# crowsonkb/k-diffusion

Hardware: NVIDIA H100
Metric: images/sec (256x256, Heun 50-step) (higher is better)
Workload: dtype bf16

## Files before the change

__graft_entry__.py:

```python
import os
import subprocess
import sys
from pathlib import Path

ROOT = Path(__file__).resolve().parent
PKG = ROOT / "k-diffusion_b200"
for p in (str(ROOT), str(PKG)):
    if p not in sys.path:
        sys.path.insert(0, p)


def build():
    env = dict(os.environ)
    env["PATH"] = os.path.join(env.get("CUDA_HOME", "/usr/local/cuda"), "bin") + os.pathsep + env.get("PATH", "")
    subprocess.run(["make", "-C", str(PKG / "csrc"), "-j8"], check=True, env=env)
    import k_diffusion
    from k_diffusion import _native
    lib = _native.lib()
    assert lib.kdb_abi_version() == _native.ABI_VERSION
    print(f"built {_native.LIB_PATH} (ABI {_native.ABI_VERSION}, {len(_native.SIGNATURES)} symbols bound)")


def smoke():
    import json
# ... 4 lines not shown
    from oracle import kdiff_oracle as O
    from oracle.fixtures import assert_close, synth_sd

    assert torch.cuda.is_available(), "smoke() needs a GPU"
    meta = json.loads((ROOT / "tests/golden/cfg1_mnist_shapes.json").read_text())
    cfg = K.config.load_config(meta["config"])
    sd = synth_sd(meta["shapes"], 1)
    inner = K.config.make_model(cfg)
    inner.load_state_dict(sd)
    inner = inner.to("cuda:0").eval().set_precision("fp32")
    model = K.config.make_denoiser_wrapper(cfg)(inner)
    g = torch.Generator().manual_seed(0)
    x = torch.randn(2, 1, 28, 28, generator=g) * 80
    cc = torch.tensor([3, 10])
    sigmas = K.sampling.get_sigmas_karras(3, 1e-2, 80)
    want = O.sample_heun(O.make_denoiser(sd, cfg["model"]), x, sigmas, dict(class_cond=cc))
    n0 = K.sampling.total_kernel_launches()
    got = K.sampling.sample_heun(model, x.cuda(), sigmas.cuda(), extra_args=dict(class_cond=cc.cuda()), disable=True)
    torch.cuda.synchronize()
    assert_close(got, want, what="smoke: sample_heun vs oracle")
    inner.set_precision("bf16")
    b = model(x.cuda(), torch.tensor([1.0, 5.0], device="cuda"), class_cond=cc.cuda())
    assert torch.isfinite(b).all()
    meta = json.loads((ROOT / "tests/golden/sw64_shapes.json").read_text())
    budget = json.loads((ROOT / "tests/golden/bf16_budget.json").read_text())["sw64_heun6"]["rel_l2"]
    cfg2 = K.config.load_config(meta["config"])
    sd2 = synth_sd(meta["shapes"], 1)
    inner2 = K.config.make_model(cfg2)
    inner2.load_state_dict(sd2)
    model2 = K.config.make_denoiser_wrapper(cfg2)(inner2.to("cuda:0").eval().set_precision("bf16"))
    g = torch.Generator().manual_seed(124)
# ... 15 lines not shown
```

k-diffusion_b200/csrc/tc_common.cuh:

```cuda
#pragma once
#include <cuda.h>

#include "common.cuh"
#include "pipe_state.cuh"

namespace kdb {
namespace tc {

__device__ __forceinline__ uint32_t smem_u32(const void* p) { return (uint32_t)__cvta_generic_to_shared(p); }

__device__ __forceinline__ void pdl_wait() { asm volatile("griddepcontrol.wait;" ::: "memory"); }

__device__ __forceinline__ uint8_t* smem_1k() {
  extern __shared__ uint8_t smem_raw[];
  return reinterpret_cast<uint8_t*>((reinterpret_cast<uintptr_t>(smem_raw) + 1023) & ~(uintptr_t)1023);
}
__device__ __forceinline__ int tiles_owned(int tiles) {
  return (int)blockIdx.x < tiles ? (tiles - 1 - (int)blockIdx.x) / (int)gridDim.x + 1 : 0;
}

__device__ __forceinline__ void mbar_init(uint64_t* bar, uint32_t count) {
  asm volatile("mbarrier.init.shared::cta.b64 [%0], %1;" ::"r"(smem_u32(bar)), "r"(count));
}
__device__ __forceinline__ void fence_barrier_init() { asm volatile("fence.mbarrier_init.release.cluster;" ::: "memory"); }
// ... 43 lines not shown
                   smem_u32(smem_dst)),
               "l"(reinterpret_cast<uint64_t>(map)), "r"(smem_u32(bar)), "r"(c0), "r"(c1), "r"(c2)
               : "memory");
}
__device__ __forceinline__ void tma_load_4d(void* smem_dst, const CUtensorMap* map, uint64_t* bar, int c0, int c1, int c2, int c3) {
  asm volatile("cp.async.bulk.tensor.4d.shared::cluster.global.mbarrier::complete_tx::bytes [%0], [%1, {%3, %4, %5, %6}], [%2];" ::"r"(
                   smem_u32(smem_dst)),
               "l"(reinterpret_cast<uint64_t>(map)), "r"(smem_u32(bar)), "r"(c0), "r"(c1), "r"(c2), "r"(c3)
               : "memory");
}

__device__ __forceinline__ void tma_load_5d(void* smem_dst, const CUtensorMap* map, uint64_t* bar, int c0, int c1, int c2, int c3, int c4) {
  asm volatile("cp.async.bulk.tensor.5d.shared::cluster.global.mbarrier::complete_tx::bytes [%0], [%1, {%3, %4, %5, %6, %7}], [%2];" ::"r"(
                   smem_u32(smem_dst)),
               "l"(reinterpret_cast<uint64_t>(map)), "r"(smem_u32(bar)), "r"(c0), "r"(c1), "r"(c2), "r"(c3), "r"(c4)
               : "memory");
}
__device__ __forceinline__ void tma_store_4d(const CUtensorMap* map, const void* smem_src, int c0, int c1, int c2, int c3) {
  asm volatile("cp.async.bulk.tensor.4d.global.shared::cta.bulk_group [%0, {%2, %3, %4, %5}], [%1];" ::"l"(reinterpret_cast<uint64_t>(map)),
               "r"(smem_u32(smem_src)), "r"(c0), "r"(c1), "r"(c2), "r"(c3)
               : "memory");
}
__device__ __forceinline__ void tma_store_3d(const CUtensorMap* map, const void* smem_src, int c0, int c1, int c2) {
  asm volatile("cp.async.bulk.tensor.3d.global.shared::cta.bulk_group [%0, {%2, %3, %4}], [%1];" ::"l"(reinterpret_cast<uint64_t>(map)),
               "r"(smem_u32(smem_src)), "r"(c0), "r"(c1), "r"(c2)
               : "memory");
}
__device__ __forceinline__ void tma_store_2d(const CUtensorMap* map, const void* smem_src, int c0, int c1) {
  asm volatile("cp.async.bulk.tensor.2d.global.shared::cta.bulk_group [%0, {%2, %3}], [%1];" ::"l"(reinterpret_cast<uint64_t>(map)),
               "r"(smem_u32(smem_src)), "r"(c0), "r"(c1)
// ... 160 lines not shown
      "{\n\t.reg .pred p;\n\t"
      "elect.sync _|p, 0xffffffff;\n\t"
      "selp.u32 %0, 1, 0, p;\n\t}"
      : "=r"(pred));
  return pred != 0;
}

__device__ __forceinline__ uint32_t pack_bf16x2(float lo, float hi) {
  __nv_bfloat162 t = __floats2bfloat162_rn(lo, hi);
  return *reinterpret_cast<uint32_t*>(&t);
}
__device__ __forceinline__ void unpack_bf16x2(uint32_t v, float& lo, float& hi) {
  __nv_bfloat162 t = *reinterpret_cast<__nv_bfloat162*>(&v);
  lo = __low2float(t);
  hi = __high2float(t);
}

__device__ __forceinline__ void window_coords(int win, int h, int w, int& b, int& wi, int& wj) {
  const int nww = w >> 3, per_img = (h >> 3) * nww;
  b = win / per_img;
  const int rem = win - b * per_img;
  wi = rem / nww;
  wj = rem - wi * nww;
}
__device__ __forceinline__ void quad_origin(int wi, int wj, int q, int h, int w, int shift, int& r, int& c) {
  r = (wi * 8 + (q >> 1) * 4 - shift + h) % h;
  c = (wj * 8 + (q & 1) * 4 - shift + w) % w;
}
__device__ __forceinline__ bool seam_ok(int qq, int kq, bool seam_r, bool seam_c) {
  return (!seam_r || ((kq >> 1) == (qq >> 1))) && (!seam_c || ((kq & 1) == (qq & 1)));
// ... 129 lines not shown
```

k-diffusion_b200/csrc/tc_ffn_fused.cuh:

```cuda
#pragma once

constexpr int FF_C = 128;
constexpr int FF_CH = 64;
constexpr int FF_XBUF = 2, FF_WU = 3, FF_WD = 3;
constexpr int FF_X_BYTES = 2 * A_STAGE_BYTES;
constexpr int FF_WU_BYTES = 2 * A_STAGE_BYTES;
constexpr int FF_WD_BYTES = A_STAGE_BYTES;
constexpr int FF_THREADS = 256 + 128;

struct FfnBars {
  tc::TmaRing<FF_XBUF> x;
  tc::TmaRing<FF_WU> wu;
  tc::TmaRing<FF_WD> wd;
};
constexpr size_t FF_SMEM = (size_t)FF_XBUF * FF_X_BYTES + (size_t)FF_WU * FF_WU_BYTES + (size_t)FF_WD * FF_WD_BYTES + sizeof(FfnBars) + 1024;

struct FfnParams {
  const float* ss_in;
  float* ss_out;
  int64_t M;
  int nc;
};

__global__ void __launch_bounds__(FF_THREADS, 1) ffn_fused_kernel(const __grid_constant__ CUtensorMap tmx, const __grid_constant__ CUtensorMap tmwu,
// ... 64 lines not shown
    const uint32_t xa = tc::smem_u32(sX + (size_t)xs.slot * FF_X_BYTES) + (uint32_t)wg * 8192u;
#pragma unroll
    for (int j = 0; j < 64; ++j) acc2[j] = 0.f;
    for (int c = 0; c <= nc; ++c) {
      if (c > 0) {
        tc::wg_wait<0>();
        tc::wg_fence_acc(acc1);
        tc::wg_fence_acc(acc2);
        tc::wg_fence_acc(hreg);
        if (lane == 0) bars->wu.release(us);
        us.advance();
        if (c > 1) {
          if (lane == 0) bars->wd.release(ds);
          ds.advance();
        }
#pragma unroll
        for (int q = 0; q < 8; ++q) {
          const tc::f32x2 v0 = tc::mul2(tc::pk2(acc1[8 * q], acc1[8 * q + 1]), h0), v1 = tc::mul2(tc::pk2(acc1[8 * q + 2], acc1[8 * q + 3]), h1);
          const tc::f32x2 q0 = tc::mul2(tc::pk2(acc1[8 * q + 4], acc1[8 * q + 5]), g0), q1 = tc::mul2(tc::pk2(acc1[8 * q + 6], acc1[8 * q + 7]), g1);
          float o0, o1, o2, o3;
          tc::upk2(tc::geglu2(v0, q0), o0, o1);
          tc::upk2(tc::geglu2(v1, q1), o2, o3);
          hreg[(q >> 1) * 4 + (q & 1) * 2 + 0] = tc::pack_bf16x2(o0, o1);
          hreg[(q >> 1) * 4 + (q & 1) * 2 + 1] = tc::pack_bf16x2(o2, o3);
        }
      }
#pragma unroll
      for (int j = 0; j < 64; ++j) acc1[j] = 0.f;
      tc::wg_fence_acc(acc1);
      if (wg == 1) tc::named_barrier_sync(tc::BAR_TURN + 1, 256);
      else if (!first_block) tc::named_barrier_sync(tc::BAR_TURN, 256);
      first_block = false;
      if (c > 0) {
        bars->wd.wait(ds);
        const uint64_t bd = tc::smem_desc_k_sw128(wd_base + ds.slot * (uint32_t)FF_WD_BYTES);
        tc::wg_fence_acc(acc2);
        tc::wg_fence_acc(hreg);
        tc::wg_fence();
#pragma unroll
        for (int kk = 0; kk < 4; ++kk) {
// ... 61 lines not shown
```

k-diffusion_b200/csrc/tc_kernels.cu:

```cuda
#include "tc_common.cuh"
#include "tc_kernels.cuh"

namespace kdb {

typedef CUresult (*EncodeTiledFn)(CUtensorMap*, CUtensorMapDataType, cuuint32_t, void*, const cuuint64_t*, const cuuint64_t*,
                                  const cuuint32_t*, const cuuint32_t*, CUtensorMapInterleave, CUtensorMapSwizzle,
                                  CUtensorMapL2promotion, CUtensorMapFloatOOBfill);

static EncodeTiledFn encode_fn() {
  static EncodeTiledFn fn = [] {
    void* p = nullptr;
    cudaDriverEntryPointQueryResult q;
    if (cudaGetDriverEntryPoint("cuTensorMapEncodeTiled", &p, cudaEnableDefault, &q) != cudaSuccess) p = nullptr;
    return reinterpret_cast<EncodeTiledFn>(p);
  }();
  return fn;
}

int make_tmap_bf16(CUtensorMap* out, const void* base, int rank, const uint64_t* dims, const uint64_t* strides_bytes, const uint32_t* box) {
  EncodeTiledFn fn = encode_fn();
  KDB_REQUIRE(fn != nullptr, KDB_ERR_UNSUPPORTED, "cuTensorMapEncodeTiled not available from this driver");
  cuuint64_t gd[5];
  cuuint64_t gs[5];
  cuuint32_t bx[5], es[5];
// ... 20 lines not shown

bool pdl_enabled() {
  static const bool enabled = [] {
    const char* e = getenv("KDB200_NO_PDL");
    return !(e != nullptr && e[0] == '1');
  }();
  return enabled;
}

namespace {

constexpr int BM = 128, BK = 64;
constexpr int A_STAGE_BYTES = BM * BK * 2;
constexpr int SUB_TILE_BYTES = BM * 128;
constexpr int GEMM_THREADS = 384;
constexpr int GEMM_RING_BYTES = 96 * 1024;

struct GemmArgs : GemmEpi {
  bf16* out;
  int64_t M;
  int N, K;
  int box_w, box_h;
  int th, tw;
};

__device__ __forceinline__ float bf16_round(float v) { return __bfloat162float(__float2bfloat16_rn(v)); }

int tmap_2d(CUtensorMap* t, const void* base, uint64_t inner, uint64_t outer, uint32_t box_inner, uint32_t box_outer) {
  const uint64_t dims[2] = {inner, outer};
  const uint64_t strides[1] = {inner * 2};
  const uint32_t box[2] = {box_inner, box_outer};
// ... 8 lines not shown
}

bool quad_box(int wc, int* box_w, int* box_h) {
  if (wc >= BM) {
    if (wc % BM != 0) return false;
    *box_w = BM;
    *box_h = 1;
    return true;
  }
  if (BM % wc != 0) return false;
  *box_w = wc;
  *box_h = BM / wc;
  return true;
}

template <int BN, int EPI> constexpr int out_bytes() {
  return EPI == EPI_GEGLU ? SUB_TILE_BYTES : (EPI == EPI_SPLIT_LERP || EPI == EPI_PATCH_OUT) ? 0 : (BN / 64) * SUB_TILE_BYTES;
}
template <int BN, int EPI> constexpr size_t gemm_smem() { return 1024 + GEMM_RING_BYTES + BM * BN * 4 + 2 * out_bytes<BN, EPI>() + 128; }

template <int BN> __device__ __forceinline__ int stage_off(int row, int chunk) { return row * BN + ((chunk ^ (row & 7)) << 2); }
template <int BN>
__device__ __forceinline__ void stage_store(float* s, int row0, const float (&d)[BN / 2]) {
  const int t = threadIdx.x & 127;
  const int r = row0 + 16 * (t >> 5) + ((t & 31) >> 2), c = 2 * (t & 3);
#pragma unroll
  for (int j = 0; j < BN / 8; ++j) {
    *reinterpret_cast<float2*>(s + stage_off<BN>(r, 2 * j + (c >> 2)) + (c & 3)) = make_float2(d[4 * j], d[4 * j + 1]);
    *reinterpret_cast<float2*>(s + stage_off<BN>(r + 8, 2 * j + (c >> 2)) + (c & 3)) = make_float2(d[4 * j + 2], d[4 * j + 3]);
  }
}
template <int BN>
__device__ __forceinline__ void stage_ld32(const float* s, int row, int col0, float (&v)[32]) {
#pragma unroll
// ... 1 lines not shown
    const float4 q = *reinterpret_cast<const float4*>(s + stage_off<BN>(row, (col0 >> 2) + i));
    v[4 * i] = q.x;
    v[4 * i + 1] = q.y;
    v[4 * i + 2] = q.z;
    v[4 * i + 3] = q.w;
  }
}

template <int BN, int EPI>
__global__ void __launch_bounds__(GEMM_THREADS, 1) gemm_wg_kernel(const __grid_constant__ CUtensorMap tma, const __grid_constant__ CUtensorMap tmb,
                                                                  const __grid_constant__ CUtensorMap tmc, const __grid_constant__ CUtensorMap tmr,
                                                                  const GemmArgs p) {
  KDB_PDL_TRIGGER();
  constexpr int B_STAGE_BYTES = BN * BK * 2;
  constexpr int STAGE_BYTES = A_STAGE_BYTES + B_STAGE_BYTES;
  constexpr int STAGES = GEMM_RING_BYTES / STAGE_BYTES;
  constexpr int NSUB = BN / 64;
  constexpr bool RES = EPI == EPI_RESID;
  uint8_t* base = tc::smem_1k();
  float* sAcc = reinterpret_cast<float*>(base + GEMM_RING_BYTES);
  auto* ring = reinterpret_cast<tc::TmaRing<STAGES>*>(base + GEMM_RING_BYTES + BM * BN * 4 + 2 * out_bytes<BN, EPI>());
  uint64_t* resid_full = reinterpret_cast<uint64_t*>(ring + 1);

  const int warp = threadIdx.x >> 5, lane = threadIdx.x & 31;
  const int nkb = p.K / BK;
  const int n_tiles = p.N / BN;
  const int n_local = tc::tiles_owned((int)((p.M + BM - 1) / BM) * n_tiles);

  if (threadIdx.x == 0) {
    tc::tma_prefetch_desc(&tma);
    tc::tma_prefetch_desc(&tmb);
    ring->init(tc::REL_WARPS);
    tc::mbar_init(&resid_full[0], 1);
    tc::mbar_init(&resid_full[1], 1);
    tc::fence_barrier_init();
  }
// ... 1 lines not shown
  tc::pdl_wait();

  if (warp >= 8) {
    tc::setmaxnreg_dec<tc::PRODUCER_REGS>();
    if (warp == 8 && tc::elect_one()) {
      int it = 0;
      for (int i = 0; i < n_local; ++i) {
        const int t = (int)blockIdx.x + i * (int)gridDim.x;
        const int64_t m0 = (int64_t)(t / n_tiles) * BM;
        const int n0 = (t % n_tiles) * BN;
        for (int kb = 0; kb < nkb; ++kb, ++it) {
          const auto ps = PipeState<STAGES>::at(it);
          uint64_t* bar = ring->acquire(ps, STAGE_BYTES);
          uint8_t* a = base + (size_t)ps.slot * STAGE_BYTES;
          if (p.mC > 0) {
            const int qd = (kb * BK) / p.mC, e0 = kb * BK - qd * p.mC;
            tc::tma_load_5d(a, &tma, bar, e0, qd & 1, p.box_h == 1 ? (int)(m0 % p.mwc) : 0, qd >> 1, (int)(m0 / p.mwc));
          } else {
            tc::tma_load_2d(a, &tma, bar, kb * BK, (int)m0);
          }
          tc::tma_load_2d(a + A_STAGE_BYTES, &tmb, bar, kb * BK, n0);
        }
      }
    }
    return;
  }
  tc::setmaxnreg_inc<tc::MMA_REGS>();

  const int wg = warp >> 2;
  const int row = threadIdx.x & 127;
  uint8_t* sC = base + GEMM_RING_BYTES + BM * BN * 4 + wg * out_bytes<BN, EPI>();
  for (int i = wg; i < n_local; i += 2) {
    const int t = (int)blockIdx.x + i * (int)gridDim.x;
    const int64_t m0 = (int64_t)(t / n_tiles) * BM;
    const int n0 = (t % n_tiles) * BN;
    if constexpr (RES) {
      if (row == 0) {
        tc::mbar_arrive_expect_tx(&resid_full[wg], NSUB * SUB_TILE_BYTES);
#pragma unroll
        for (int g = 0; g < NSUB; ++g) tc::tma_load_2d(sC + g * SUB_TILE_BYTES, &tmr, &resid_full[wg], n0 + g * 64, (int)m0);
      }
    }

    float acc0[BN / 2], acc1[BN / 2];
#pragma unroll
    for (int k = 0; k < BN / 2; ++k) acc0[k] = acc1[k] = 0.f;
    if (i > 0) tc::named_barrier_sync(tc::BAR_TURN + wg, 256);
    const int it0 = i * nkb;
    for (int kb = 0; kb < nkb; ++kb) {
      const auto ps = PipeState<STAGES>::at(it0 + kb);
      ring->wait(ps);
      const uint32_t a_addr = tc::smem_u32(base + (size_t)ps.slot * STAGE_BYTES);
      const uint64_t ad0 = tc::smem_desc_k_sw128(a_addr), ad1 = tc::smem_desc_k_sw128(a_addr + 8 * 1024);
      const uint64_t bd = tc::smem_desc_k_sw128(a_addr + A_STAGE_BYTES);
      tc::wg_fence_acc(acc0);
// ... 8 lines not shown
          tc::wgmma_64<0>(acc0, ad0 + 2ull * k, bd + 2ull * k, 1u);
          tc::wgmma_64<0>(acc1, ad1 + 2ull * k, bd + 2ull * k, 1u);
        }
      }
      tc::wg_commit();
      tc::wg_wait<1>();
      tc::wg_fence_acc(acc0);
      tc::wg_fence_acc(acc1);
      if (kb > 0 && lane == 0) ring->release(PipeState<STAGES>::at(it0 + kb - 1));
    }
    if (i + 1 < n_local) tc::named_barrier_arrive(tc::BAR_TURN + (wg ^ 1), 256);
    tc::wg_wait<0>();
    tc::wg_fence_acc(acc0);
    tc::wg_fence_acc(acc1);
    if (lane == 0) ring->release(PipeState<STAGES>::at(it0 + nkb - 1));
    if (i > 0) tc::named_barrier_sync(tc::BAR_ACC + wg, 256);
    stage_store<BN>(sAcc, 0, acc0);
    stage_store<BN>(sAcc, 64, acc1);
    tc::named_barrier_sync(tc::BAR_WG + wg, 128);
    const bool pass_acc = i + 1 < n_local;

    const int64_t m = m0 + row;
    float rstd = 1.f;
    if (p.ss_in != nullptr) {
      const float4* sp = reinterpret_cast<const float4*>(p.ss_in + (m < p.M ? m : 0) * SS_PARTS);
      rstd = rsqrtf(tc::rowss_sum(__ldg(sp), __ldg(sp + 1), p.K >> 7) / (float)p.K + 1e-6f);
    }
    if constexpr (EPI == EPI_PATCH_OUT) {
      float v[64];
      {
// ... 22 lines not shown
            const int64_t o = (((int64_t)b * 3 + c) * p.H + (ty * 4 + nh)) * p.W + tx * 4;
            float4 y = make_float4(bf16_round(v[(nh * 4 + 0) * 3 + c]), bf16_round(v[(nh * 4 + 1) * 3 + c]), bf16_round(v[(nh * 4 + 2) * 3 + c]),
                                   bf16_round(v[(nh * 4 + 3) * 3 + c]));
            if (p.sigma_data > 0.f) {
              const float4 xi = __ldg(reinterpret_cast<const float4*>(p.x_in + o));
              y = make_float4(y.x * c_out + xi.x * c_skip, y.y * c_out + xi.y * c_skip, y.z * c_out + xi.z * c_skip, y.w * c_out + xi.w * c_skip);
            }
            *reinterpret_cast<float4*>(p.img + o) = y;
          }
      }
    } else if constexpr (EPI == EPI_SPLIT_LERP) {
      const bool live = m < p.M;
      const float facv = __ldg(p.fac);
      float ss = 0.f;
      int64_t fine = 0;
#pragma unroll 1
      for (int c = 0; c < BN / 32; ++c) {
        float v[32];
        stage_ld32<BN>(sAcc, row, c * 32, v);
        if (c == BN / 32 - 1 && pass_acc) tc::named_barrier_arrive(tc::BAR_ACC + (wg ^ 1), 256);
        if (!live) continue;
        const int n = n0 + c * 32;
        const int64_t b = m / ((int64_t)p.hc * p.wc);
        const int r = (int)(m - b * p.hc * p.wc);
        const int hy = r / p.wc, wx = r - hy * p.wc;
        const int qd = n / p.C, e = n - qd * p.C;
        fine = (b * (2 * p.hc) + (2 * hy + (qd >> 1))) * (2 * p.wc) + (2 * wx + (qd & 1));
        const int64_t off = fine * p.C + e;
        const uint4* sk = reinterpret_cast<const uint4*>(static_cast<const bf16*>(p.resid) + off);
        uint4* dst = reinterpret_cast<uint4*>(p.out + off);
// ... 18 lines not shown
      if (p.ss_out != nullptr && live) p.ss_out[fine * SS_PARTS + ((n0 % p.C) >> 7)] = ss;
    } else {
      if constexpr (RES) tc::mbar_wait_nocall(&resid_full[wg], (uint32_t)(i >> 1) & 1u);
      float ss_acc[4] = {0.f, 0.f, 0.f, 0.f};
#pragma unroll 1
      for (int g = 0; g < NSUB; ++g) {
        float v[64];
        {
          float t0[32], t1[32];
          stage_ld32<BN>(sAcc, row, g * 64, t0);
          stage_ld32<BN>(sAcc, row, g * 64 + 32, t1);
#pragma unroll
          for (int k = 0; k < 32; ++k) { v[k] = t0[k]; v[32 + k] = t1[k]; }
        }
        if (g == NSUB - 1 && pass_acc) tc::named_barrier_arrive(tc::BAR_ACC + (wg ^ 1), 256);
        if (EPI != EPI_GEGLU && p.ss_in != nullptr) {
          bool apply = true;
          if constexpr (EPI == EPI_QKV_ROPE) apply = (n0 + g * 64) >= 2 * p.C;
          if (apply) {
#pragma unroll
            for (int k = 0; k < 64; ++k) v[k] *= rstd;
          }
        }
        if constexpr (EPI == EPI_GEGLU) {
          const tc::f32x2 r2 = tc::pk2(rstd, rstd), rh = tc::pk2(0.5f * rstd, 0.5f * rstd);
#pragma unroll
          for (int gg = 0; gg < 4; ++gg) {
            uint32_t o[4];
#pragma unroll
            for (int j = 0; j < 4; ++j) {
              tc::f32x2 val = tc::pk2(v[gg * 16 + 2 * j], v[gg * 16 + 2 * j + 1]);
              tc::f32x2 gate = tc::pk2(v[gg * 16 + 8 + 2 * j], v[gg * 16 + 8 + 2 * j + 1]);
              val = tc::mul2(val, rh);
              if (p.ss_in != nullptr) gate = tc::mul2(gate, r2);
              float o0, o1;
              tc::upk2(tc::geglu2(val, gate), o0, o1);
              o[j] = tc::pack_bf16x2(o0, o1);
            }
            *reinterpret_cast<uint4*>(sC + tc::sw128_offset(row, g * 4 + gg)) = make_uint4(o[0], o[1], o[2], o[3]);
          }
        } else {
          uint8_t* cg = sC + g * SUB_TILE_BYTES;
          if constexpr (RES) {
#pragma unroll
            for (int j = 0; j < 8; ++j) {
              const uint4 r4 = *reinterpret_cast<const uint4*>(cg + tc::sw128_offset(row, j));
              const uint32_t rw[4] = {r4.x, r4.y, r4.z, r4.w};
#pragma unroll
              for (int q = 0; q < 4; ++q) {
                v[j * 8 + q * 2] += __uint_as_float(rw[q] << 16);
                v[j * 8 + q * 2 + 1] += __uint_as_float(rw[q] & 0xffff0000u);
              }
            }
          }
          if constexpr (RES || EPI == EPI_STORE) {
            if (p.ss_out != nullptr) {
#pragma unroll
              for (int k = 0; k < 64; k += 4) {
                ss_acc[0] = fmaf(v[k], v[k], ss_acc[0]);
                ss_acc[1] = fmaf(v[k + 1], v[k + 1], ss_acc[1]);
                ss_acc[2] = fmaf(v[k + 2], v[k + 2], ss_acc[2]);
                ss_acc[3] = fmaf(v[k + 3], v[k + 3], ss_acc[3]);
              }
            }
          }
          if constexpr (EPI == EPI_QKV_ROPE) {
            const int n = n0 + g * 64;
            const int t3 = n / p.C, head = (n - t3 * p.C) >> 6;
            if (t3 < 2) {
              const int64_t tok = (m < p.M ? m : 0) % p.T_tokens;
              const float4* tb = reinterpret_cast<const float4*>(p.rope) + (int64_t)head * 8 * p.T_tokens + tok;
              tc::f32x2 P[32];
#pragma unroll
              for (int k = 0; k < 32; ++k) P[k] = tc::pk2(v[2 * k], v[2 * k + 1]);
              tc::f32x2 q0 = tc::mul2(P[0], P[0]), q1 = tc::mul2(P[1], P[1]), q2 = tc::mul2(P[2], P[2]), q3 = tc::mul2(P[3], P[3]);
#pragma unroll
              for (int k = 4; k < 32; k += 4) {
                q0 = tc::fma2(P[k], P[k], q0);
                q1 = tc::fma2(P[k + 1], P[k + 1], q1);
                q2 = tc::fma2(P[k + 2], P[k + 2], q2);
                q3 = tc::fma2(P[k + 3], P[k + 3], q3);
              }
              const float sc = sqrtf(__ldg(p.qk_scale + head)) * rsqrtf(((q0.x + q0.y) + (q1.x + q1.y)) + ((q2.x + q2.y) + (q3.x + q3.y)) + 1e-6f);
              const tc::f32x2 sc2 = tc::pk2(sc, sc);
#pragma unroll
              for (int k = 0; k < 8; ++k) {
                const float4 cs = __ldg(tb + (int64_t)k * p.T_tokens);
                const tc::f32x2 C = tc::pk2(cs.x, cs.y), S = tc::pk2(cs.z, cs.w);
                const tc::f32x2 X1 = P[k], X2 = P[8 + k];
                P[k] = tc::mul2(tc::fma2(X2, tc::neg2(S), tc::mul2(X1, C)), sc2);
                P[8 + k] = tc::mul2(tc::fma2(X1, S, tc::mul2(X2, C)), sc2);
              }
#pragma unroll
              for (int k = 16; k < 32; ++k) P[k] = tc::mul2(P[k], sc2);
#pragma unroll
              for (int k = 0; k < 32; ++k) tc::upk2(P[k], v[2 * k], v[2 * k + 1]);
            }
          }
#pragma unroll
          for (int j = 0; j < 8; ++j)
            *reinterpret_cast<uint4*>(cg + tc::sw128_offset(row, j)) =
                make_uint4(tc::pack_bf16x2(v[j * 8 + 0], v[j * 8 + 1]), tc::pack_bf16x2(v[j * 8 + 2], v[j * 8 + 3]),
                           tc::pack_bf16x2(v[j * 8 + 4], v[j * 8 + 5]), tc::pack_bf16x2(v[j * 8 + 6], v[j * 8 + 7]));
        }
      }
      if constexpr (RES || EPI == EPI_STORE) {
        if (p.ss_out != nullptr && m < p.M) p.ss_out[m * SS_PARTS + (n0 >> 7)] = (ss_acc[0] + ss_acc[1]) + (ss_acc[2] + ss_acc[3]);
      }
      tc::fence_proxy_async();
      tc::named_barrier_sync(tc::BAR_WG + wg, 128);
      if (row == 0) {
        if constexpr (EPI == EPI_GEGLU) {
          tc::tma_store_2d(&tmc, sC, n0 / 2, (int)m0);
        } else {
#pragma unroll
          for (int g = 0; g < NSUB; ++g) tc::tma_store_2d(&tmc, sC + g * SUB_TILE_BYTES, n0 + g * 64, (int)m0);
        }
        tc::tma_store_commit();
        tc::tma_store_wait_read();
      }
    }
  }
}


#include "tc_ffn_fused.cuh"
#include "tc_attn_block.cuh"

template <int BN, int EPI>
int launch_tc(const bf16* A, const bf16* W, const GemmArgs& p, cudaStream_t st) {
  CUtensorMap ta, tb, tcm, tr;
  int rc;
  if (p.mC > 0) {
    if ((rc = tmap_quad(&ta, A, p.mC, p.mwc, (uint64_t)p.M / p.mwc, p.box_w, p.box_h))) return rc;
  } else {
    if ((rc = tmap_2d(&ta, A, (uint64_t)p.K, (uint64_t)p.M, BK, BM))) return rc;
  }
  if ((rc = tmap_2d(&tb, W, (uint64_t)p.K, (uint64_t)p.N, BK, BN))) return rc;
  const uint64_t n_out = EPI == EPI_GEGLU ? (uint64_t)p.N / 2 : (uint64_t)p.N;
  if (EPI != EPI_SPLIT_LERP && EPI != EPI_PATCH_OUT) {
    if ((rc = tmap_2d(&tcm, p.out, n_out, (uint64_t)p.M, 64, BM))) return rc;
  } else {
    tcm = ta;
  }
  if (EPI == EPI_RESID) {
    if ((rc = tmap_2d(&tr, p.resid, (uint64_t)p.N, (uint64_t)p.M, 64, BM))) return rc;
  } else {
    tr = ta;
  }
  constexpr size_t smem = gemm_smem<BN, EPI>();
  static_assert(smem <= 227 * 1024, "GEMM shared memory exceeds the 227 KiB opt-in limit");
  static bool opened = false;
  if ((rc = set_smem_once(gemm_wg_kernel<BN, EPI>, opened, (int)smem))) return rc;
  KDB_CUDA(launch_pdl(gemm_wg_kernel<BN, EPI>, persistent_grid(ceil_div(p.M, BM) * (p.N / BN)), dim3(GEMM_THREADS), smem, st, ta, tb, tcm, tr, p));
  KDB_LAUNCH_CHECK(EPI == EPI_PATCH_OUT ? F_PATCH_OUT : F_GEMM_TC, st);
  return 0;
}

template <int EPI>
int dispatch_bn(const bf16* A, const bf16* W, const GemmArgs& p, cudaStream_t st) {
  if (p.N % 128 == 0) return launch_tc<128, EPI>(A, W, p, st);
  return launch_tc<64, EPI>(A, W, p, st);
}
// ... 202 lines not shown
  KDB_REQUIRE(aligned16(A) && aligned16(W) && aligned16(C), KDB_ERR_BAD_ARG, "gemm_tc: operands must be 16-byte aligned");
  KDB_REQUIRE(gemm_fits(M, N, K, epi), KDB_ERR_UNSUPPORTED, "gemm_tc: epilogue %d does not support M=%lld N=%d K=%d with these options", epi.mode,
              (long long)M, N, K);
  GemmArgs p{};
  static_cast<GemmEpi&>(p) = epi;
  p.out = C;
  p.M = M;
  p.N = N;
  p.K = K;
  p.th = epi.H / 4;
  p.tw = epi.W / 4;
  if (epi.mC > 0) {
    quad_box(epi.mwc, &p.box_w, &p.box_h);
    return launch_tc<128, EPI_STORE>(A, W, p, st);
  }
  switch (epi.mode) {
    case EPI_STORE:
      return dispatch_bn<EPI_STORE>(A, W, p, st);
    case EPI_RESID:
      return dispatch_bn<EPI_RESID>(A, W, p, st);
    case EPI_GEGLU:
      return launch_tc<128, EPI_GEGLU>(A, W, p, st);
    case EPI_SPLIT_LERP:
      return dispatch_bn<EPI_SPLIT_LERP>(A, W, p, st);
    case EPI_QKV_ROPE:
      return dispatch_bn<EPI_QKV_ROPE>(A, W, p, st);
    case EPI_PATCH_OUT:
      return launch_tc<64, EPI_PATCH_OUT>(A, W, p, st);
    default:
      return KDB_ERR_BAD_ARG;
// ... 126 lines not shown
```

Baseline: 126.2.

## Apply GEGLU from registers and add TMA-based split-lerp epilogue

The GEGLU GEMM epilogue now computes the gated activation straight from the MMA accumulator fragments, with per-row rstd preloaded. This skips the fp32 shared-memory accumulator staging and frees that space for a doubled TMA ring with more pipeline stages. A new SPLIT_LERP path loads the residual and stores the output through 5D quad-layout TMA maps into swizzled shared memory, replacing the previous per-thread global accesses. The extra stages and TMA paths raise shared-memory and register pressure and add layout-dependent indexing that must match the quad unpatching.

```diff
diff --git a/__graft_entry__.py b/__graft_entry__.py
--- a/__graft_entry__.py
+++ b/__graft_entry__.py
@@ -42,7 +42,8 @@
     x = torch.randn(2, 1, 28, 28, generator=g) * 80
     cc = torch.tensor([3, 10])
     sigmas = K.sampling.get_sigmas_karras(3, 1e-2, 80)
-    want = O.sample_heun(O.make_denoiser(sd, cfg["model"]), x, sigmas, dict(class_cond=cc))
+    sd64 = {k: (v.double() if v.is_floating_point() else v) for k, v in sd.items()}
+    want = O.sample_heun(O.make_denoiser(sd64, cfg["model"]), x.double(), sigmas.double(), dict(class_cond=cc))
     n0 = K.sampling.total_kernel_launches()
     got = K.sampling.sample_heun(model, x.cuda(), sigmas.cuda(), extra_args=dict(class_cond=cc.cuda()), disable=True)
     torch.cuda.synchronize()
diff --git a/k-diffusion_b200/csrc/tc_common.cuh b/k-diffusion_b200/csrc/tc_common.cuh
--- a/k-diffusion_b200/csrc/tc_common.cuh
+++ b/k-diffusion_b200/csrc/tc_common.cuh
@@ -81,6 +81,11 @@
   asm volatile("cp.async.bulk.tensor.5d.shared::cluster.global.mbarrier::complete_tx::bytes [%0], [%1, {%3, %4, %5, %6, %7}], [%2];" ::"r"(
                    smem_u32(smem_dst)),
                "l"(reinterpret_cast<uint64_t>(map)), "r"(smem_u32(bar)), "r"(c0), "r"(c1), "r"(c2), "r"(c3), "r"(c4)
+               : "memory");
+}
+__device__ __forceinline__ void tma_store_5d(const CUtensorMap* map, const void* smem_src, int c0, int c1, int c2, int c3, int c4) {
+  asm volatile("cp.async.bulk.tensor.5d.global.shared::cta.bulk_group [%0, {%2, %3, %4, %5, %6}], [%1];" ::"l"(reinterpret_cast<uint64_t>(map)),
+               "r"(smem_u32(smem_src)), "r"(c0), "r"(c1), "r"(c2), "r"(c3), "r"(c4)
                : "memory");
 }
 __device__ __forceinline__ void tma_store_4d(const CUtensorMap* map, const void* smem_src, int c0, int c1, int c2, int c3) {
@@ -271,6 +276,19 @@
   __nv_bfloat162 t = *reinterpret_cast<__nv_bfloat162*>(&v);
   lo = __low2float(t);
   hi = __high2float(t);
+}
+
+__device__ __forceinline__ void geglu_fragment(const float (&acc)[64], f32x2 h0, f32x2 h1, f32x2 g0, f32x2 g1, uint32_t (&o)[16]) {
+#pragma unroll
+  for (int q = 0; q < 8; ++q) {
+    const f32x2 v0 = mul2(pk2(acc[8 * q], acc[8 * q + 1]), h0), v1 = mul2(pk2(acc[8 * q + 2], acc[8 * q + 3]), h1);
+    const f32x2 q0 = mul2(pk2(acc[8 * q + 4], acc[8 * q + 5]), g0), q1 = mul2(pk2(acc[8 * q + 6], acc[8 * q + 7]), g1);
+    float o0, o1, o2, o3;
+    upk2(geglu2(v0, q0), o0, o1);
+    upk2(geglu2(v1, q1), o2, o3);
+    o[2 * q] = pack_bf16x2(o0, o1);
+    o[2 * q + 1] = pack_bf16x2(o2, o3);
+  }
 }
 
 __device__ __forceinline__ void window_coords(int win, int h, int w, int& b, int& wi, int& wj) {
diff --git a/k-diffusion_b200/csrc/tc_ffn_fused.cuh b/k-diffusion_b200/csrc/tc_ffn_fused.cuh
--- a/k-diffusion_b200/csrc/tc_ffn_fused.cuh
+++ b/k-diffusion_b200/csrc/tc_ffn_fused.cuh
@@ -102,16 +102,7 @@
           if (lane == 0) bars->wd.release(ds);
           ds.advance();
         }
-#pragma unroll
-        for (int q = 0; q < 8; ++q) {
-          const tc::f32x2 v0 = tc::mul2(tc::pk2(acc1[8 * q], acc1[8 * q + 1]), h0), v1 = tc::mul2(tc::pk2(acc1[8 * q + 2], acc1[8 * q + 3]), h1);
-          const tc::f32x2 q0 = tc::mul2(tc::pk2(acc1[8 * q + 4], acc1[8 * q + 5]), g0), q1 = tc::mul2(tc::pk2(acc1[8 * q + 6], acc1[8 * q + 7]), g1);
-          float o0, o1, o2, o3;
-          tc::upk2(tc::geglu2(v0, q0), o0, o1);
-          tc::upk2(tc::geglu2(v1, q1), o2, o3);
-          hreg[(q >> 1) * 4 + (q & 1) * 2 + 0] = tc::pack_bf16x2(o0, o1);
-          hreg[(q >> 1) * 4 + (q & 1) * 2 + 1] = tc::pack_bf16x2(o2, o3);
-        }
+        tc::geglu_fragment(acc1, h0, h1, g0, g1, hreg);
       }
 #pragma unroll
       for (int j = 0; j < 64; ++j) acc1[j] = 0.f;
diff --git a/k-diffusion_b200/csrc/tc_kernels.cu b/k-diffusion_b200/csrc/tc_kernels.cu
--- a/k-diffusion_b200/csrc/tc_kernels.cu
+++ b/k-diffusion_b200/csrc/tc_kernels.cu
@@ -58,7 +58,6 @@
 constexpr int A_STAGE_BYTES = BM * BK * 2;
 constexpr int SUB_TILE_BYTES = BM * 128;
 constexpr int GEMM_THREADS = 384;
-constexpr int GEMM_RING_BYTES = 96 * 1024;
 
 struct GemmArgs : GemmEpi {
   bf16* out;
@@ -97,10 +96,20 @@
   return true;
 }
 
+struct QuadCoord {
+  int e, nw, wx, nh, row;
+};
+__device__ __forceinline__ QuadCoord quad_coord(int64_t m0, int n, int C, int wc, int box_h) {
+  const int qd = n / C;
+  return QuadCoord{n - qd * C, qd & 1, box_h == 1 ? (int)(m0 % wc) : 0, qd >> 1, (int)(m0 / wc)};
+}
+
 template <int BN, int EPI> constexpr int out_bytes() {
-  return EPI == EPI_GEGLU ? SUB_TILE_BYTES : (EPI == EPI_SPLIT_LERP || EPI == EPI_PATCH_OUT) ? 0 : (BN / 64) * SUB_TILE_BYTES;
-}
-template <int BN, int EPI> constexpr size_t gemm_smem() { return 1024 + GEMM_RING_BYTES + BM * BN * 4 + 2 * out_bytes<BN, EPI>() + 128; }
+  return EPI == EPI_GEGLU ? SUB_TILE_BYTES : EPI == EPI_PATCH_OUT ? 0 : (BN / 64) * SUB_TILE_BYTES;
+}
+template <int BN, int EPI> constexpr int acc_bytes() { return EPI == EPI_GEGLU ? 0 : BM * BN * 4; }
+template <int EPI> constexpr int ring_bytes() { return EPI == EPI_GEGLU ? 192 * 1024 : 96 * 1024; }
+template <int BN, int EPI> constexpr size_t gemm_smem() { return 1024 + ring_bytes<EPI>() + acc_bytes<BN, EPI>() + 2 * out_bytes<BN, EPI>() + 128; }
 
 template <int BN> __device__ __forceinline__ int stage_off(int row, int chunk) { return row * BN + ((chunk ^ (row & 7)) << 2); }
 template <int BN>
@@ -132,12 +141,13 @@
   KDB_PDL_TRIGGER();
   constexpr int B_STAGE_BYTES = BN * BK * 2;
   constexpr int STAGE_BYTES = A_STAGE_BYTES + B_STAGE_BYTES;
-  constexpr int STAGES = GEMM_RING_BYTES / STAGE_BYTES;
+  constexpr int RING_BYTES = ring_bytes<EPI>();
+  constexpr int STAGES = RING_BYTES / STAGE_BYTES;
   constexpr int NSUB = BN / 64;
   constexpr bool RES = EPI == EPI_RESID;
   uint8_t* base = tc::smem_1k();
-  float* sAcc = reinterpret_cast<float*>(base + GEMM_RING_BYTES);
-  auto* ring = reinterpret_cast<tc::TmaRing<STAGES>*>(base + GEMM_RING_BYTES + BM * BN * 4 + 2 * out_bytes<BN, EPI>());
+  float* sAcc = reinterpret_cast<float*>(base + RING_BYTES);
+  auto* ring = reinterpret_cast<tc::TmaRing<STAGES>*>(base + RING_BYTES + acc_bytes<BN, EPI>() + 2 * out_bytes<BN, EPI>());
   uint64_t* resid_full = reinterpret_cast<uint64_t*>(ring + 1);
 
   const int warp = threadIdx.x >> 5, lane = threadIdx.x & 31;
@@ -169,8 +179,8 @@
           uint64_t* bar = ring->acquire(ps, STAGE_BYTES);
           uint8_t* a = base + (size_t)ps.slot * STAGE_BYTES;
           if (p.mC > 0) {
-            const int qd = (kb * BK) / p.mC, e0 = kb * BK - qd * p.mC;
-            tc::tma_load_5d(a, &tma, bar, e0, qd & 1, p.box_h == 1 ? (int)(m0 % p.mwc) : 0, qd >> 1, (int)(m0 / p.mwc));
+            const QuadCoord q = quad_coord(m0, kb * BK, p.mC, p.mwc, p.box_h);
+            tc::tma_load_5d(a, &tma, bar, q.e, q.nw, q.wx, q.nh, q.row);
           } else {
             tc::tma_load_2d(a, &tma, bar, kb * BK, (int)m0);
           }
@@ -184,16 +194,35 @@
 
   const int wg = warp >> 2;
   const int row = threadIdx.x & 127;
-  uint8_t* sC = base + GEMM_RING_BYTES + BM * BN * 4 + wg * out_bytes<BN, EPI>();
+  uint8_t* sC = base + RING_BYTES + acc_bytes<BN, EPI>() + wg * out_bytes<BN, EPI>();
+  const int r0 = 16 * (warp & 3) + (lane >> 2), cq = 2 * (lane & 3);
   for (int i = wg; i < n_local; i += 2) {
     const int t = (int)blockIdx.x + i * (int)gridDim.x;
     const int64_t m0 = (int64_t)(t / n_tiles) * BM;
     const int n0 = (t % n_tiles) * BN;
-    if constexpr (RES) {
-      if (row == 0) {
+    if constexpr (RES || EPI == EPI_SPLIT_LERP) {
+      if (row == 0 && (RES || p.box_w > 0)) {
         tc::mbar_arrive_expect_tx(&resid_full[wg], NSUB * SUB_TILE_BYTES);
 #pragma unroll
-        for (int g = 0; g < NSUB; ++g) tc::tma_load_2d(sC + g * SUB_TILE_BYTES, &tmr, &resid_full[wg], n0 + g * 64, (int)m0);
+        for (int g = 0; g < NSUB; ++g) {
+          if constexpr (RES) {
+            tc::tma_load_2d(sC + g * SUB_TILE_BYTES, &tmr, &resid_full[wg], n0 + g * 64, (int)m0);
+          } else {
+            const QuadCoord q = quad_coord(m0, n0 + g * 64, p.C, p.wc, p.box_h);
+            tc::tma_load_5d(sC + g * SUB_TILE_BYTES, &tmr, &resid_full[wg], q.e, q.nw, q.wx, q.nh, q.row);
+          }
+        }
+      }
+    }
+    float frag_rstd[4] = {1.f, 1.f, 1.f, 1.f};
+    if constexpr (EPI == EPI_GEGLU) {
+      if (p.ss_in != nullptr) {
+#pragma unroll
+        for (int h = 0; h < 4; ++h) {
+          const int64_t m = m0 + r0 + 64 * (h >> 1) + 8 * (h & 1);
+          const float4* sp = reinterpret_cast<const float4*>(p.ss_in + (m < p.M ? m : 0) * SS_PARTS);
+          frag_rstd[h] = rsqrtf(tc::rowss_sum(__ldg(sp), __ldg(sp + 1), p.K >> 7) / (float)p.K + 1e-6f);
+        }
       }
     }
 
@@ -232,6 +261,31 @@
     tc::wg_fence_acc(acc0);
     tc::wg_fence_acc(acc1);
     if (lane == 0) ring->release(PipeState<STAGES>::at(it0 + nkb - 1));
+
+    if constexpr (EPI == EPI_GEGLU) {
+      tc::named_barrier_sync(tc::BAR_WG + wg, 128);
+#pragma unroll
+      for (int half = 0; half < 2; ++half) {
+        const float r_a = frag_rstd[2 * half], r_b = frag_rstd[2 * half + 1];
+        uint32_t o[16];
+        tc::geglu_fragment(half == 0 ? acc0 : acc1, tc::pk2(0.5f * r_a, 0.5f * r_a), tc::pk2(0.5f * r_b, 0.5f * r_b), tc::pk2(r_a, r_a),
+                           tc::pk2(r_b, r_b), o);
+        const int r = 64 * half + r0;
+#pragma unroll
+        for (int q = 0; q < 8; ++q) {
+          *reinterpret_cast<uint32_t*>(sC + tc::sw128_offset(r, q) + 2 * cq) = o[2 * q];
+          *reinterpret_cast<uint32_t*>(sC + tc::sw128_offset(r + 8, q) + 2 * cq) = o[2 * q + 1];
+        }
+      }
+      tc::fence_proxy_async();
+      tc::named_barrier_sync(tc::BAR_WG + wg, 128);
+      if (row == 0) {
+        tc::tma_store_2d(&tmc, sC, n0 / 2, (int)m0);
+        tc::tma_store_commit();
+        tc::tma_store_wait_read();
+      }
+      continue;
+    }
     if (i > 0) tc::named_barrier_sync(tc::BAR_ACC + wg, 256);
     stage_store<BN>(sAcc, 0, acc0);
     stage_store<BN>(sAcc, 64, acc1);
@@ -284,6 +338,59 @@
       const float facv = __ldg(p.fac);
       float ss = 0.f;
       int64_t fine = 0;
+      if (p.box_w > 0) {
+        tc::mbar_wait_nocall(&resid_full[wg], (uint32_t)(i >> 1) & 1u);
+#pragma unroll 1
+        for (int g = 0; g < NSUB; ++g) {
+          float v[64];
+          {
+            float t0[32], t1[32];
+            stage_ld32<BN>(sAcc, row, g * 64, t0);
+            stage_ld32<BN>(sAcc, row, g * 64 + 32, t1);
+#pragma unroll
+            for (int k = 0; k < 32; ++k) { v[k] = t0[k]; v[32 + k] = t1[k]; }
+          }
+          if (g == NSUB - 1 && pass_acc) tc::named_barrier_arrive(tc::BAR_ACC + (wg ^ 1), 256);
+          uint8_t* cg = sC + g * SUB_TILE_BYTES;
+#pragma unroll
+          for (int j = 0; j < 8; ++j) {
+            uint4* cp = reinterpret_cast<uint4*>(cg + tc::sw128_offset(row, j));
+            const uint4 r4 = *cp;
+            const uint32_t rw[4] = {r4.x, r4.y, r4.z, r4.w};
+            uint32_t ow[4];
+#pragma unroll
+            for (int q = 0; q < 4; ++q) {
+              const float lo = __uint_as_float(rw[q] << 16), hi = __uint_as_float(rw[q] & 0xffff0000u);
+              const float e0 = v[j * 8 + q * 2], e1 = v[j * 8 + q * 2 + 1];
+              const float d0 = e0 - lo, d1 = e1 - hi;
+              const float o0 = (facv < 0.5f) ? fmaf(facv, d0, lo) : e0 - d0 * (1.f - facv);
+              const float o1 = (facv < 0.5f) ? fmaf(facv, d1, hi) : e1 - d1 * (1.f - facv);
+              ss = fmaf(o0, o0, fmaf(o1, o1, ss));
+              ow[q] = tc::pack_bf16x2(o0, o1);
+            }
+            *cp = make_uint4(ow[0], ow[1], ow[2], ow[3]);
+          }
+        }
+        if (p.ss_out != nullptr && live) {
+          const int64_t b = m / ((int64_t)p.hc * p.wc);
+          const int r = (int)(m - b * p.hc * p.wc);
+          const int hy = r / p.wc, wx = r - hy * p.wc, qd = n0 / p.C;
+          fine = (b * (2 * p.hc) + (2 * hy + (qd >> 1))) * (2 * p.wc) + (2 * wx + (qd & 1));
+          p.ss_out[fine * SS_PARTS + ((n0 % p.C) >> 7)] = ss;
+        }
+        tc::fence_proxy_async();
+        tc::named_barrier_sync(tc::BAR_WG + wg, 128);
+        if (row == 0) {
+#pragma unroll
+          for (int g = 0; g < NSUB; ++g) {
+            const QuadCoord q = quad_coord(m0, n0 + g * 64, p.C, p.wc, p.box_h);
+            tc::tma_store_5d(&tmc, sC + g * SUB_TILE_BYTES, q.e, q.nw, q.wx, q.nh, q.row);
+          }
+          tc::tma_store_commit();
+          tc::tma_store_wait_read();
+        }
+        continue;
+      }
 #pragma unroll 1
       for (int c = 0; c < BN / 32; ++c) {
         float v[32];
@@ -332,7 +439,7 @@
           for (int k = 0; k < 32; ++k) { v[k] = t0[k]; v[32 + k] = t1[k]; }
         }
         if (g == NSUB - 1 && pass_acc) tc::named_barrier_arrive(tc::BAR_ACC + (wg ^ 1), 256);
-        if (EPI != EPI_GEGLU && p.ss_in != nullptr) {
+        if (p.ss_in != nullptr) {
           bool apply = true;
           if constexpr (EPI == EPI_QKV_ROPE) apply = (n0 + g * 64) >= 2 * p.C;
           if (apply) {
@@ -340,87 +447,68 @@
             for (int k = 0; k < 64; ++k) v[k] *= rstd;
           }
         }
-        if constexpr (EPI == EPI_GEGLU) {
-          const tc::f32x2 r2 = tc::pk2(rstd, rstd), rh = tc::pk2(0.5f * rstd, 0.5f * rstd);
-#pragma unroll
-          for (int gg = 0; gg < 4; ++gg) {
-            uint32_t o[4];
-#pragma unroll
-            for (int j = 0; j < 4; ++j) {
-              tc::f32x2 val = tc::pk2(v[gg * 16 + 2 * j], v[gg * 16 + 2 * j + 1]);
-              tc::f32x2 gate = tc::pk2(v[gg * 16 + 8 + 2 * j], v[gg * 16 + 8 + 2 * j + 1]);
-              val = tc::mul2(val, rh);
-              if (p.ss_in != nullptr) gate = tc::mul2(gate, r2);
-              float o0, o1;
-              tc::upk2(tc::geglu2(val, gate), o0, o1);
-              o[j] = tc::pack_bf16x2(o0, o1);
+        uint8_t* cg = sC + g * SUB_TILE_BYTES;
+        if constexpr (RES) {
+#pragma unroll
+          for (int j = 0; j < 8; ++j) {
+            const uint4 r4 = *reinterpret_cast<const uint4*>(cg + tc::sw128_offset(row, j));
+            const uint32_t rw[4] = {r4.x, r4.y, r4.z, r4.w};
+#pragma unroll
+            for (int q = 0; q < 4; ++q) {
+              v[j * 8 + q * 2] += __uint_as_float(rw[q] << 16);
+              v[j * 8 + q * 2 + 1] += __uint_as_float(rw[q] & 0xffff0000u);
             }
-            *reinterpret_cast<uint4*>(sC + tc::sw128_offset(row, g * 4 + gg)) = make_uint4(o[0], o[1], o[2], o[3]);
-          }
-        } else {
-          uint8_t* cg = sC + g * SUB_TILE_BYTES;
-          if constexpr (RES) {
-#pragma unroll
-            for (int j = 0; j < 8; ++j) {
-              const uint4 r4 = *reinterpret_cast<const uint4*>(cg + tc::sw128_offset(row, j));
-              const uint32_t rw[4] = {r4.x, r4.y, r4.z, r4.w};
-#pragma unroll
-              for (int q = 0; q < 4; ++q) {
-                v[j * 8 + q * 2] += __uint_as_float(rw[q] << 16);
-                v[j * 8 + q * 2 + 1] += __uint_as_float(rw[q] & 0xffff0000u);
-              }
+          }
+        }
+        if constexpr (RES || EPI == EPI_STORE) {
+          if (p.ss_out != nullptr) {
+#pragma unroll
+            for (int k = 0; k < 64; k += 4) {
+              ss_acc[0] = fmaf(v[k], v[k], ss_acc[0]);
+              ss_acc[1] = fmaf(v[k + 1], v[k + 1], ss_acc[1]);
+              ss_acc[2] = fmaf(v[k + 2], v[k + 2], ss_acc[2]);
+              ss_acc[3] = fmaf(v[k + 3], v[k + 3], ss_acc[3]);
             }
           }
-          if constexpr (RES || EPI == EPI_STORE) {
-            if (p.ss_out != nullptr) {
-#pragma unroll
-              for (int k = 0; k < 64; k += 4) {
-                ss_acc[0] = fmaf(v[k], v[k], ss_acc[0]);
-                ss_acc[1] = fmaf(v[k + 1], v[k + 1], ss_acc[1]);
-                ss_acc[2] = fmaf(v[k + 2], v[k + 2], ss_acc[2]);
-                ss_acc[3] = fmaf(v[k + 3], v[k + 3], ss_acc[3]);
-              }
+        }
+        if constexpr (EPI == EPI_QKV_ROPE) {
+          const int n = n0 + g * 64;
+          const int t3 = n / p.C, head = (n - t3 * p.C) >> 6;
+          if (t3 < 2) {
+            const int64_t tok = (m < p.M ? m : 0) % p.T_tokens;
+            const float4* tb = reinterpret_cast<const float4*>(p.rope) + (int64_t)head * 8 * p.T_tokens + tok;
+            tc::f32x2 P[32];
+#pragma unroll
+            for (int k = 0; k < 32; ++k) P[k] = tc::pk2(v[2 * k], v[2 * k + 1]);
+            tc::f32x2 q0 = tc::mul2(P[0], P[0]), q1 = tc::mul2(P[1], P[1]), q2 = tc::mul2(P[2], P[2]), q3 = tc::mul2(P[3], P[3]);
+#pragma unroll
+            for (int k = 4; k < 32; k += 4) {
+              q0 = tc::fma2(P[k], P[k], q0);
+              q1 = tc::fma2(P[k + 1], P[k + 1], q1);
+              q2 = tc::fma2(P[k + 2], P[k + 2], q2);
+              q3 = tc::fma2(P[k + 3], P[k + 3], q3);
             }
-          }
-          if constexpr (EPI == EPI_QKV_ROPE) {
-            const int n = n0 + g * 64;
-            const int t3 = n / p.C, head = (n - t3 * p.C) >> 6;
-            if (t3 < 2) {
-              const int64_t tok = (m < p.M ? m : 0) % p.T_tokens;
-              const float4* tb = reinterpret_cast<const float4*>(p.rope) + (int64_t)head * 8 * p.T_tokens + tok;
-              tc::f32x2 P[32];
-#pragma unroll
-              for (int k = 0; k < 32; ++k) P[k] = tc::pk2(v[2 * k], v[2 * k + 1]);
-              tc::f32x2 q0 = tc::mul2(P[0], P[0]), q1 = tc::mul2(P[1], P[1]), q2 = tc::mul2(P[2], P[2]), q3 = tc::mul2(P[3], P[3]);
-#pragma unroll
-              for (int k = 4; k < 32; k += 4) {
-                q0 = tc::fma2(P[k], P[k], q0);
-                q1 = tc::fma2(P[k + 1], P[k + 1], q1);
-                q2 = tc::fma2(P[k + 2], P[k + 2], q2);
-                q3 = tc::fma2(P[k + 3], P[k + 3], q3);
-              }
-              const float sc = sqrtf(__ldg(p.qk_scale + head)) * rsqrtf(((q0.x + q0.y) + (q1.x + q1.y)) + ((q2.x + q2.y) + (q3.x + q3.y)) + 1e-6f);
-              const tc::f32x2 sc2 = tc::pk2(sc, sc);
-#pragma unroll
-              for (int k = 0; k < 8; ++k) {
-                const float4 cs = __ldg(tb + (int64_t)k * p.T_tokens);
-                const tc::f32x2 C = tc::pk2(cs.x, cs.y), S = tc::pk2(cs.z, cs.w);
-                const tc::f32x2 X1 = P[k], X2 = P[8 + k];
-                P[k] = tc::mul2(tc::fma2(X2, tc::neg2(S), tc::mul2(X1, C)), sc2);
-                P[8 + k] = tc::mul2(tc::fma2(X1, S, tc::mul2(X2, C)), sc2);
-              }
-#pragma unroll
-              for (int k = 16; k < 32; ++k) P[k] = tc::mul2(P[k], sc2);
-#pragma unroll
-              for (int k = 0; k < 32; ++k) tc::upk2(P[k], v[2 * k], v[2 * k + 1]);
+            const float sc = sqrtf(__ldg(p.qk_scale + head)) * rsqrtf(((q0.x + q0.y) + (q1.x + q1.y)) + ((q2.x + q2.y) + (q3.x + q3.y)) + 1e-6f);
+            const tc::f32x2 sc2 = tc::pk2(sc, sc);
+#pragma unroll
+            for (int k = 0; k < 8; ++k) {
+              const float4 cs = __ldg(tb + (int64_t)k * p.T_tokens);
+              const tc::f32x2 C = tc::pk2(cs.x, cs.y), S = tc::pk2(cs.z, cs.w);
+              const tc::f32x2 X1 = P[k], X2 = P[8 + k];
+              P[k] = tc::mul2(tc::fma2(X2, tc::neg2(S), tc::mul2(X1, C)), sc2);
+              P[8 + k] = tc::mul2(tc::fma2(X1, S, tc::mul2(X2, C)), sc2);
             }
-          }
-#pragma unroll
-          for (int j = 0; j < 8; ++j)
-            *reinterpret_cast<uint4*>(cg + tc::sw128_offset(row, j)) =
-                make_uint4(tc::pack_bf16x2(v[j * 8 + 0], v[j * 8 + 1]), tc::pack_bf16x2(v[j * 8 + 2], v[j * 8 + 3]),
-                           tc::pack_bf16x2(v[j * 8 + 4], v[j * 8 + 5]), tc::pack_bf16x2(v[j * 8 + 6], v[j * 8 + 7]));
-        }
+#pragma unroll
+            for (int k = 16; k < 32; ++k) P[k] = tc::mul2(P[k], sc2);
+#pragma unroll
+            for (int k = 0; k < 32; ++k) tc::upk2(P[k], v[2 * k], v[2 * k + 1]);
+          }
+        }
+#pragma unroll
+        for (int j = 0; j < 8; ++j)
+          *reinterpret_cast<uint4*>(cg + tc::sw128_offset(row, j)) =
+              make_uint4(tc::pack_bf16x2(v[j * 8 + 0], v[j * 8 + 1]), tc::pack_bf16x2(v[j * 8 + 2], v[j * 8 + 3]),
+                         tc::pack_bf16x2(v[j * 8 + 4], v[j * 8 + 5]), tc::pack_bf16x2(v[j * 8 + 6], v[j * 8 + 7]));
       }
       if constexpr (RES || EPI == EPI_STORE) {
         if (p.ss_out != nullptr && m < p.M) p.ss_out[m * SS_PARTS + (n0 >> 7)] = (ss_acc[0] + ss_acc[1]) + (ss_acc[2] + ss_acc[3]);
@@ -428,12 +516,8 @@
       tc::fence_proxy_async();
       tc::named_barrier_sync(tc::BAR_WG + wg, 128);
       if (row == 0) {
-        if constexpr (EPI == EPI_GEGLU) {
-          tc::tma_store_2d(&tmc, sC, n0 / 2, (int)m0);
-        } else {
-#pragma unroll
-          for (int g = 0; g < NSUB; ++g) tc::tma_store_2d(&tmc, sC + g * SUB_TILE_BYTES, n0 + g * 64, (int)m0);
-        }
+#pragma unroll
+        for (int g = 0; g < NSUB; ++g) tc::tma_store_2d(&tmc, sC + g * SUB_TILE_BYTES, n0 + g * 64, (int)m0);
         tc::tma_store_commit();
         tc::tma_store_wait_read();
       }
@@ -456,15 +540,20 @@
   }
   if ((rc = tmap_2d(&tb, W, (uint64_t)p.K, (uint64_t)p.N, BK, BN))) return rc;
   const uint64_t n_out = EPI == EPI_GEGLU ? (uint64_t)p.N / 2 : (uint64_t)p.N;
-  if (EPI != EPI_SPLIT_LERP && EPI != EPI_PATCH_OUT) {
-    if ((rc = tmap_2d(&tcm, p.out, n_out, (uint64_t)p.M, 64, BM))) return rc;
+  if (EPI == EPI_SPLIT_LERP && p.box_w > 0) {
+    if ((rc = tmap_quad(&tcm, p.out, p.C, p.wc, (uint64_t)p.M / p.wc, p.box_w, p.box_h))) return rc;
+    if ((rc = tmap_quad(&tr, p.resid, p.C, p.wc, (uint64_t)p.M / p.wc, p.box_w, p.box_h))) return rc;
   } else {
-    tcm = ta;
-  }
-  if (EPI == EPI_RESID) {
-    if ((rc = tmap_2d(&tr, p.resid, (uint64_t)p.N, (uint64_t)p.M, 64, BM))) return rc;
-  } else {
-    tr = ta;
+    if (EPI != EPI_SPLIT_LERP && EPI != EPI_PATCH_OUT) {
+      if ((rc = tmap_2d(&tcm, p.out, n_out, (uint64_t)p.M, 64, BM))) return rc;
+    } else {
+      tcm = ta;
+    }
+    if (EPI == EPI_RESID) {
+      if ((rc = tmap_2d(&tr, p.resid, (uint64_t)p.N, (uint64_t)p.M, 64, BM))) return rc;
+    } else {
+      tr = ta;
+    }
   }
   constexpr size_t smem = gemm_smem<BN, EPI>();
   static_assert(smem <= 227 * 1024, "GEMM shared memory exceeds the 227 KiB opt-in limit");
@@ -697,6 +786,7 @@
     quad_box(epi.mwc, &p.box_w, &p.box_h);
     return launch_tc<128, EPI_STORE>(A, W, p, st);
   }
+  if (epi.mode == EPI_SPLIT_LERP && epi.C % 64 == 0 && epi.wc > 0 && M % epi.wc == 0 && aligned16(epi.resid)) quad_box(epi.wc, &p.box_w, &p.box_h);
   switch (epi.mode) {
     case EPI_STORE:
       return dispatch_bn<EPI_STORE>(A, W, p, st);
```

After: 132.0 (median of 6 runs). +4.6%, better.
